# xuyuan/waymo_2d_tracking

Hardware: AMD Instinct MI355X
Metric: end-to-end frames/sec (detect+SORT) on 1920x1280 Waymo frames (higher is better)
Workload: dtype f32; 1 GPU; Cascade R-CNN X152-32x8d-FPN dconv (random-init, fp32, batch 1) on synthetic 1920x1280x3 frames -> top-100 detections/frame -> SORT (max_age 2, min_hits 0, all boxes tracked; trackers resident for the whole segment); 5 cameras x 2 frames per step per GPU; 1x1 and dense 3x3 convolutions: f32 operands as exact 3 x bf16 splits, six cross terms on the bf16 matrix cores, f32 accumulate (csrc/det_gemm_s; stage=e2e, parallelism=sequence-shard x1

## Files before the change

include/waymodet.h:

```cpp
#ifndef WAYMODET_H
#define WAYMODET_H
#include <stddef.h>
#include <stdint.h>
#ifdef __cplusplus
extern "C" {
#endif

int wd_roi_pool_fpn_f32(const float* const* feats, const int32_t* heights, const int32_t* widths,
                        const float* scales, int n_levels, int channels, int batch,
                        const float* rois, int n_rois, int pooled, int min_level, int canonical_level,
                        float canonical_size, float* out, void* stream);

size_t wd_nms_workspace(int n);
int wd_select_kept(const uint8_t* keep_mask, const uint8_t* valid, const int64_t* order, int n, int cap, int64_t* out_idx,
                   int32_t* count, void* stream);
int wd_nms_sorted_f32(const float* boxes, const int32_t* idxs, int n, float iou_threshold,
                      uint8_t* keep_mask, int32_t* n_keep, void* workspace, size_t workspace_bytes, void* stream);

size_t wd_gemm_nt_workspace(int M, int N, int K);
int wd_gemm_nt_ws_f32(const float* A, const float* Bt, const float* bias, const float* residual, int relu, int M, int N, int K,
                      float* C, void* workspace, size_t workspace_bytes, void* stream);

int wd_gemm_lt_f32(const float* a, const float* w, const float* bias, const float* residual, float* out, int m, int n, int k,
                   int relu, void* workspace, size_t workspace_bytes, void* stream);
int wd_gemm_lt_plan_info(int m, int n, int k, int relu, int has_bias, int has_residual, float* best_us, int* candidates);
size_t wd_gemm_split_packed_bytes(int N, int K);
int wd_gemm_split_pack_weight(const float* w, int N, int K, void* packed, void* stream);
int wd_gemm_split_pack_weight_strided(const float* w, int N, int K, long stride_n, long stride_k, void* packed, void* stream);
typedef struct WdSplitPackDesc {
    const float* src;
    void* dst;
    long s_n, s_c, s_kh, s_kw;
    long first_block;
    int N, K, C, ksize, flip, reserved;
} WdSplitPackDesc;
int wd_gemm_split_pack_batch(const WdSplitPackDesc* descs_device, int count, long total_blocks, void* stream);
size_t wd_gemm_split_workspace(long M, int N, int K);
int wd_gemm_split_f32(const float* a, long lda, const void* packed_w, const float* bias, const float* residual, float* out, long ldc,
                      int M, int N, int K, int relu, void* workspace, size_t workspace_bytes, void* stream);
int wd_conv_split_f32(const float* x, int batch, int H, int W, int C, const void* packed_w, int ksize, int stride, int pad, const float* bias,
                      const float* residual, float* out, int N, int relu, void* workspace, size_t workspace_bytes, void* stream);
int wd_gemm_split_supported(const float* a, long lda, const float* bias, const float* residual, const float* out, long ldc, long M, int N, int K);
int wd_conv_split_position_major(int batch, int H, int W, int ksize, int stride, int pad);
typedef struct WdSplitIO {
    const float* a;
    long lda;
    const void* a_planes;
    const float* residual;
    const void* residual_planes;
    float* out;
    void* out_planes;
    long ldc;
} WdSplitIO;
size_t wd_split_planes_bytes(long M, int K);
int wd_split_planes_pack_f32(const float* a, long lda, long M, int K, void* planes, void* stream);
int wd_split_planes_unpack_f32(const void* planes, long M, int K, float* out, long ldo, void* stream);
int wd_gemm_split_io(const WdSplitIO* io, const void* packed_w, const float* bias, int M, int N, int K, int relu, void* workspace,
                     size_t workspace_bytes, void* stream);
int wd_nms_segmented_f32(const float* boxes, const int32_t* idxs, const int32_t* seg_offsets, int n_seg, float iou_threshold,
                         uint8_t* keep_mask, int32_t* n_keep, void* workspace, size_t workspace_bytes, void* stream);

size_t wd_rpn_topk_workspace(const int* n_per_level, int n_levels, int k);
int wd_rpn_topk_decode_f32(const float* const* logits, const float* const* deltas, const float* const* anchors,
                           const int* n_per_level, int n_levels, int k, float img_h, float img_w, float scale_clamp,
                           float* out_boxes, float* out_scores, int32_t* out_group, uint8_t* out_valid, void* workspace,
                           size_t workspace_bytes, void* stream);
int wd_sort_candidates_f32(const float* boxes, const float* scores, const int32_t* group, const uint8_t* valid,
                           const uint8_t* valid2 , int n, float* out_boxes, float* out_scores, int32_t* out_group, uint8_t* out_valid, int64_t* out_order,
                           void* stream);
int wd_box_candidates_f32(const float* boxes, const float* s0, const float* s1, const float* s2, const int32_t* n_valid, int rows,
                          int num_classes, float score_thresh, float img_h, float img_w, float* out_boxes, float* out_scores,
                          int32_t* out_group, uint8_t* out_valid, int64_t* out_order, void* stream);
int wd_gather_kept_f32(const uint8_t* keep, const uint8_t* valid, const float* boxes, const float* scores, const int64_t* order,
                       int n, int cap, int num_classes, float* out_boxes, float* out_scores, int64_t* out_class, int32_t* count,
                       void* stream);
int wd_detections_to_wire(const float* boxes, const float* scores, const int64_t* classes, const int32_t* count, int n, int in_w,
                          int in_h, int hflip, int out_w, int out_h, double* xywhs, int32_t* category, void* stream);

size_t wd_deform_packed_weight_floats(int c_in, int c_out, int groups);
int wd_deform_pack_weight(const float* weight_oihw, int c_in, int c_out, int groups, float* packed, void* stream);
const char* wd_deform_conv3x3_variant(int c_in, int groups, int stride, int pad, int has_offset);
const char* wd_deform_conv3x3_last_kernel(void);
int wd_deform_conv3x3_f32(const float* x, const float* offset, const float* mask, const float* packed_weight,
                          const float* scale, const float* bias, int relu,
                          int batch, int h, int w, int c_in, int c_out, int groups, int stride, int pad,
                          float* y, void* stream);
int wd_deform_conv3x3_hint_f32(const float* x, const float* offset, const float* mask, const float* packed_weight,
                               const float* scale, const float* bias, int relu, int batch, int h, int w, int c_in,
                               int c_out, int groups, int stride, int pad, int far_offsets, float* y, void* stream);
size_t wd_deform_table_bytes(int batch, int h, int w);
int wd_deform_offsets_table_f32(const float* partial, int ld, const float* bias, int batch, int h, int w, float* offsets,
                                void* table, void* stream);
int wd_deform_conv3x3_tab_f32(const float* x, const float* offset, const float* mask, const float* packed_weight,
                              const float* scale, const float* bias, int relu, int batch, int h, int w, int c_in,
                              int c_out, int groups, int stride, int pad, int far_offsets, const void* table, float* y,
                              void* stream);

int wd_gemm_nt_f32(const float* A, const float* Bt, const float* bias, const float* residual, int relu,
                   int M, int N, int K, float* C, void* stream);

int wd_groupnorm_relu_nhwc_f32(float* x, const float* gamma, const float* beta, int n, int hw, int c, int groups,
                               float eps, int relu, void* stream);
int wd_groupnorm_relu_out_nhwc_f32(const float* x, float* y, const float* gamma, const float* beta, int n, int hw, int c, int groups,
                                   float eps, int relu, void* stream);
int wd_groupnorm_relu_bwd_nhwc_f32(const float* x, const float* dy, const float* gamma, const float* beta, int n, int hw, int c, int groups,
                                   float eps, int relu, float* dx, float* dgamma, float* dbeta, void* stream);

#define WD_LAYOUT_NCHW_F32 0
#define WD_LAYOUT_NHWC_U8 1
int wd_preprocess_out_shape(int h, int w, double scale, int divisor, int* ho, int* wo, int* hp, int* wp);
int wd_preprocess_f32(const void* src, int src_layout, int batch, int h, int w, double scale, int hflip, int vflip,
                      int swap_rb, const float* mean3, const float* std3, int divisor, float* out, void* stream);

int wd_decode_boxes_f32(const float* deltas, const float* boxes, const int64_t* index, int n, float wx, float wy, float ww,
                        float wh, float scale_clamp, float clip_w, float clip_h, float* out, void* stream);

int wd_roi_pool_fpn_bwd_f32(float* const* grad_feats, const int32_t* heights, const int32_t* widths, const float* scales,
                            int n_levels, int channels, int batch, const float* rois, int n_rois, int pooled, int min_level,
                            int canonical_level, float canonical_size, const float* grad_out, void* stream);
int wd_deform_im2col_f32(const float* x, const float* offset, int batch, int h, int w, int c, int groups, int stride, int pad,
                         float* col, void* stream);
int wd_deform_col2im_f32(const float* dcol, const float* x, const float* offset, int batch, int h, int w, int c, int groups,
                         int stride, int pad, float* dx, float* doffset, void* stream);
size_t wd_deform_bwd_tables_bytes(int batch, int h, int w, int stride);
int wd_deform_dxoff_f32(const float* x, const float* offset, const float* dy, const float* y_act, const float* scale, const float* weight, int batch,
                        int h, int w, int c, int groups, int stride, unsigned char* tables, float* packed_weight, float* dx, float* doffset,
                        void* stream);
size_t wd_deform_dw_scratch_floats(int batch, int h, int w, int c, int groups, int stride);
int wd_deform_dw_f32(const float* x, const float* offset, const float* dy, const float* y_act, const float* scale, int batch, int h, int w, int c,
                     int groups, int stride, float* scratch, float* dw, void* stream);

int wd_tap_shift_add_f32(const float* partial, int ld, int n_out, const float* bias, int batch, int h, int w, int stride,
                         float* out, void* stream);

int wd_upsample2x_nhwc_f32(const float* src, int batch, int h, int w, int c, float* dst, void* stream);

int wd_bias_relu_f32(float* y, const float* bias, long m, int n, int relu, void* stream);

int wd_act_bwd_f32(const float* dy, const float* y, const float* scale, long m, int n, int relu, float* g, void* stream);

int wd_autocontrast_u8(uint8_t* img, int h, int w, void* workspace24, void* stream);

int wd_jpeg_info(const uint8_t* data, int64_t n, int32_t* width, int32_t* height, int32_t* components, int32_t* h_samp,
                 int32_t* v_samp, int32_t* restart_interval);
int wd_jpeg_decode_rgb_u8(const uint8_t* data, int64_t n, uint8_t* rgb, int64_t capacity, int32_t* width, int32_t* height,
                          int32_t* sync_rounds, void* stream);
int wd_jpeg_last_stats(int32_t* out4);

#ifdef __cplusplus
}
#endif
#endif
```

waymo_2d_tracking_amd/csrc/det_gemm_split.hip:

```cpp
#include "common.h"
#include "../../include/waymodet.h"
#include <cstdlib>
#include <cstring>

namespace {

using bf16x8 = __attribute__((ext_vector_type(8))) __bf16;
using bf16x2 = __attribute__((ext_vector_type(2))) __bf16;
using f32x2 = __attribute__((ext_vector_type(2))) float;
using f32x16 = __attribute__((ext_vector_type(16))) float;
using u32x4 = __attribute__((ext_vector_type(4))) unsigned;

constexpr int BK = 64;
constexpr int BN = 256;
constexpr int NTHREADS = 512;
constexpr int CHUNK = 6144;

struct SplitArgs {
    const float* a;
    const unsigned char* ap;
    const uint4* w;
    const float* bias;
    const float* residual;
    const unsigned char* resp;
// ... 24 lines not shown
__device__ __forceinline__ float bf_lo(unsigned v) { return __uint_as_float(v << 16); }
__device__ __forceinline__ float bf_hi(unsigned v) { return __uint_as_float(v & 0xffff0000u); }

__device__ __forceinline__ size_t planes_offset(int row, int col, int ncols) {
    return ((size_t)(row >> 5) * (size_t)(ncols >> 5) + (size_t)(col >> 5)) * CHUNK +
           (size_t)((row & 31) * 64 + ((((col >> 3) & 3) ^ ((row >> 2) & 3)) << 4) + ((col >> 2) & 1) * 8);
}

constexpr int LDC = BN + 8;

template <int MT>
__device__ __forceinline__ void split_epilogue(const SplitArgs& p, unsigned char* smem, const f32x16 (&acc)[MT], int m0, int n0, int wave, int lane, int mlim,
                                               int row_mul = 1, int row_add = 0) {
    const int rr = lane & 31, rg = lane >> 5;
    float* ct = reinterpret_cast<float*>(smem);
    const int ncols = p.N - n0 < BN ? p.N - n0 : BN;
    constexpr int PASS = 3;
    auto stage = [&](int i0) {
        if (i0 > 0) __builtin_amdgcn_s_barrier();
#pragma unroll
        for (int i = i0; i < i0 + PASS && i < MT; ++i)
#pragma unroll
            for (int e = 0; e < 16; ++e)
                ct[((i - i0) * 32 + (e & 3) + 8 * (e >> 2) + 4 * rg) * LDC + 32 * wave + rr] = acc[i][e];
        __builtin_amdgcn_s_waitcnt(0xC07F);
        __builtin_amdgcn_s_barrier();
    };
    if (p.outp == nullptr) {
        const int c4 = 4 * lane;
        float4 bv = make_float4(0.f, 0.f, 0.f, 0.f);
        if (p.bias && c4 < ncols) bv = *reinterpret_cast<const float4*>(p.bias + n0 + c4);
        constexpr int RPW = 32 * PASS / 8;
#pragma unroll
        for (int i0 = 0; i0 < MT; i0 += PASS) {
            const int nrows = 32 * ((MT - i0) < PASS ? (MT - i0) : PASS);
            float4 rv[RPW];
            if (p.residual) {
#pragma unroll
                for (int j = 0; j < RPW; ++j) {
                    const int r = wave + 8 * j, row = m0 + 32 * i0 + r;
                    rv[j] = make_float4(0.f, 0.f, 0.f, 0.f);
                    if (r < nrows && row < mlim && c4 < ncols)
                        rv[j] = *reinterpret_cast<const float4*>(p.residual + (size_t)(row * row_mul + row_add) * p.ldc + n0 + c4);
                }
            } else if (p.resp) {
#pragma unroll
                for (int j = 0; j < RPW; ++j) {
                    const int r = wave + 8 * j, row = m0 + 32 * i0 + r;
                    rv[j] = make_float4(0.f, 0.f, 0.f, 0.f);
                    if (r < nrows && row < mlim && c4 < ncols) {
                        const unsigned char* q = p.resp + planes_offset(row * row_mul + row_add, n0 + c4, p.N);
                        const uint2 h = *reinterpret_cast<const uint2*>(q), m = *reinterpret_cast<const uint2*>(q + 2048),
                                    l = *reinterpret_cast<const uint2*>(q + 4096);
                        rv[j] = make_float4((bf_lo(h.x) + bf_lo(m.x)) + bf_lo(l.x), (bf_hi(h.x) + bf_hi(m.x)) + bf_hi(l.x),
                                            (bf_lo(h.y) + bf_lo(m.y)) + bf_lo(l.y), (bf_hi(h.y) + bf_hi(m.y)) + bf_hi(l.y));
                    }
                }
            }
            stage(i0);
#pragma unroll
            for (int j = 0; j < RPW; ++j) {
                const int r = wave + 8 * j, row = m0 + 32 * i0 + r;
                if (r < nrows && row < mlim && c4 < ncols) {
                    float4 v = *reinterpret_cast<const float4*>(ct + r * LDC + c4);
                    v.x += bv.x; v.y += bv.y; v.z += bv.z; v.w += bv.w;
                    if (p.residual || p.resp) { v.x += rv[j].x; v.y += rv[j].y; v.z += rv[j].z; v.w += rv[j].w; }
                    if (p.relu) { v.x = fmaxf(v.x, 0.f); v.y = fmaxf(v.y, 0.f); v.z = fmaxf(v.z, 0.f); v.w = fmaxf(v.w, 0.f); }
                    *reinterpret_cast<float4*>(p.out + (size_t)(row * row_mul + row_add) * p.ldc + n0 + c4) = v;
                }
            }
        }
        return;
    }
    const int ur = lane >> 2;
    constexpr int UPW = PASS * 8 * 2 / 8;
    const int ncb = ncols >> 5;
#pragma unroll
    for (int i0 = 0; i0 < MT; i0 += PASS) {
        const int nrb = (MT - i0) < PASS ? (MT - i0) : PASS;
        const int nunits = nrb * ncb * 2;
        uint4 rq[UPW][3];
#pragma unroll
        for (int j = 0; j < UPW; ++j) {
            const int u = wave + 8 * j;
            rq[j][0] = rq[j][1] = rq[j][2] = make_uint4(0u, 0u, 0u, 0u);
            if (u < nunits && m0 + 32 * (i0 + u / (2 * ncb)) < mlim) {
                const int rbi = u / (2 * ncb), cb = (u >> 1) - rbi * ncb, h = u & 1;
                const int r = 16 * h + ur, row = m0 + 32 * (i0 + rbi) + r;
                const int c8 = 8 * ((lane & 3) ^ ((r >> 2) & 3)), col = n0 + 32 * cb + c8;
                if (p.resp) {
                    const unsigned char* q = p.resp + ((size_t)(row >> 5) * (size_t)(p.N >> 5) + (size_t)(col >> 5)) * CHUNK + h * 1024 + lane * 16;
                    rq[j][0] = *reinterpret_cast<const uint4*>(q);
                    rq[j][1] = *reinterpret_cast<const uint4*>(q + 2048);
                    rq[j][2] = *reinterpret_cast<const uint4*>(q + 4096);
                } else if (p.residual && row < mlim) {
                    const uint4* q = reinterpret_cast<const uint4*>(p.residual + (size_t)row * p.ldc + col);
                    rq[j][0] = q[0];
                    rq[j][1] = q[1];
                }
            }
        }
        stage(i0);
#pragma unroll
        for (int j = 0; j < UPW; ++j) {
            const int u = wave + 8 * j;
            if (u < nunits && m0 + 32 * (i0 + u / (2 * ncb)) < mlim) {
                const int rbi = u / (2 * ncb), cb = (u >> 1) - rbi * ncb, h = u & 1;
                const int r = 16 * h + ur, row = m0 + 32 * (i0 + rbi) + r;
                const int c8 = 8 * ((lane & 3) ^ ((r >> 2) & 3)), col = n0 + 32 * cb + c8;
                const float* src = ct + (32 * rbi + r) * LDC + 32 * cb + c8;
                float4 v0 = *reinterpret_cast<const float4*>(src), v1 = *reinterpret_cast<const float4*>(src + 4);
                if (p.bias) {
                    const float4 b0 = *reinterpret_cast<const float4*>(p.bias + col), b1 = *reinterpret_cast<const float4*>(p.bias + col + 4);
                    v0.x += b0.x; v0.y += b0.y; v0.z += b0.z; v0.w += b0.w; v1.x += b1.x; v1.y += b1.y; v1.z += b1.z; v1.w += b1.w;
                }
                if (p.resp) {
                    const uint4 hh = rq[j][0], mm = rq[j][1], ll = rq[j][2];
                    v0.x += (bf_lo(hh.x) + bf_lo(mm.x)) + bf_lo(ll.x); v0.y += (bf_hi(hh.x) + bf_hi(mm.x)) + bf_hi(ll.x);
                    v0.z += (bf_lo(hh.y) + bf_lo(mm.y)) + bf_lo(ll.y); v0.w += (bf_hi(hh.y) + bf_hi(mm.y)) + bf_hi(ll.y);
                    v1.x += (bf_lo(hh.z) + bf_lo(mm.z)) + bf_lo(ll.z); v1.y += (bf_hi(hh.z) + bf_hi(mm.z)) + bf_hi(ll.z);
                    v1.z += (bf_lo(hh.w) + bf_lo(mm.w)) + bf_lo(ll.w); v1.w += (bf_hi(hh.w) + bf_hi(mm.w)) + bf_hi(ll.w);
                } else if (p.residual) {
                    const uint4 q0 = rq[j][0], q1 = rq[j][1];
                    v0.x += __uint_as_float(q0.x); v0.y += __uint_as_float(q0.y); v0.z += __uint_as_float(q0.z); v0.w += __uint_as_float(q0.w);
                    v1.x += __uint_as_float(q1.x); v1.y += __uint_as_float(q1.y); v1.z += __uint_as_float(q1.z); v1.w += __uint_as_float(q1.w);
                }
                if (p.relu) {
                    v0.x = fmaxf(v0.x, 0.f); v0.y = fmaxf(v0.y, 0.f); v0.z = fmaxf(v0.z, 0.f); v0.w = fmaxf(v0.w, 0.f);
                    v1.x = fmaxf(v1.x, 0.f); v1.y = fmaxf(v1.y, 0.f); v1.z = fmaxf(v1.z, 0.f); v1.w = fmaxf(v1.w, 0.f);
                }
                if (p.out && row < mlim) {
                    float4* d = reinterpret_cast<float4*>(p.out + (size_t)row * p.ldc + col);
                    d[0] = v0; d[1] = v1;
                }
                unsigned hv[4], mv[4], lv[4];
                split_pair(v0.x, v0.y, hv[0], mv[0], lv[0]); split_pair(v0.z, v0.w, hv[1], mv[1], lv[1]);
                split_pair(v1.x, v1.y, hv[2], mv[2], lv[2]); split_pair(v1.z, v1.w, hv[3], mv[3], lv[3]);
                unsigned char* q = p.outp + ((size_t)(row >> 5) * (size_t)(p.N >> 5) + (size_t)(col >> 5)) * CHUNK + h * 1024 + lane * 16;
                *reinterpret_cast<uint4*>(q) = make_uint4(hv[0], hv[1], hv[2], hv[3]);
                *reinterpret_cast<uint4*>(q + 2048) = make_uint4(mv[0], mv[1], mv[2], mv[3]);
                *reinterpret_cast<uint4*>(q + 4096) = make_uint4(lv[0], lv[1], lv[2], lv[3]);
            }
        }
    }
}

__device__ __forceinline__ int xcd_tile_id(int total) {
    const int x = blockIdx.x & 7, j = blockIdx.x >> 3;
    const int q = total >> 3, r = total & 7;
    if (j >= q + (x < r ? 1 : 0)) return -1;
    return (x < r ? x * (q + 1) : r * (q + 1) + (x - r) * q) + j;
}

template <int MT, int MODE>
__global__ __launch_bounds__(NTHREADS, 2) void gemm_split_kernel(const SplitArgs p) {
    extern __shared__ __attribute__((aligned(16))) unsigned char smem[];
    constexpr int BM = 32 * MT;
    constexpr int PLANE = BM * 64;
    constexpr int BUF = 3 * PLANE;
    const int tid = threadIdx.x, lane = tid & 63;
    const int wave = __builtin_amdgcn_readfirstlane(tid >> 6);
    constexpr bool CONV = MODE == 1 || MODE == 3;
    constexpr bool PM = MODE == 3;
    int id = PM ? (int)blockIdx.x : xcd_tile_id(p.tiles_m * p.tiles_n * p.splitk);
    if (id < 0 || (PM && id >= p.tiles_m * p.tiles_n)) return;
#ifdef WD_DEBUG
    long long t_start = 0, r_start = 0, t_main = 0, t_epi = 0;
    if (p.stamps) { t_start = __builtin_amdgcn_s_memtime(); r_start = __builtin_amdgcn_s_memrealtime(); }
    const int id_stamp = id;
#endif
    const int kz = PM ? 0 : id % p.splitk;
    if (!PM) id /= p.splitk;
    const int tm = id / p.tiles_n, tn = id - tm * p.tiles_n;
    int m0 = tm * BM;
    const int n0 = tn * BN;
    const int kc = CONV ? p.C / 32 : 1;
    int pm_y = 0, pm_x = 0, pm_nvt = 9;
    unsigned long long pm_taps = 0x876543210ull;
    if (PM) {
        const int nch = (p.M / (p.H * p.W) + BM - 1) / BM;
        const int wi = p.W - 2, hi = p.H - 2, ni = wi * hi, ne = 2 * wi + 2 * hi;
        int t = tm, c, q;
        if (t < ni * nch) { c = t / ni; q = t - c * ni; pm_y = 1 + q / wi; pm_x = 1 + q - (q / wi) * wi; }
        else if (t < (ni + ne) * nch) {
            t -= ni * nch; c = t / ne; q = t - c * ne;
            if (q < wi) { pm_y = 0; pm_x = 1 + q; }
            else if (q < 2 * wi) { pm_y = p.H - 1; pm_x = 1 + q - wi; }
            else if (q < 2 * wi + hi) { pm_x = 0; pm_y = 1 + q - 2 * wi; }
            else { pm_x = p.W - 1; pm_y = 1 + q - 2 * wi - hi; }
        } else { t -= (ni + ne) * nch; c = t >> 2; q = t & 3; pm_y = (q >> 1) ? p.H - 1 : 0; pm_x = (q & 1) ? p.W - 1 : 0; }
        m0 = c * BM;
        pm_taps = 0; pm_nvt = 0;
        for (int tp = 0; tp < 9; ++tp) {
            const int yy = pm_y + tp / 3 - 1, xx = pm_x + tp % 3 - 1;
            if (yy >= 0 && yy < p.H && xx >= 0 && xx < p.W) { pm_taps |= (unsigned long long)tp << (4 * pm_nvt); ++pm_nvt; }
        }
    }
    auto pm_tap = [&](int i) { return (int)((pm_taps >> (4 * i)) & 15ull); };
    const int nk_all = PM ? pm_nvt * kc : p.K / 32;
    const int per = (nk_all + p.splitk - 1) / p.splitk;
    const int k0 = kz * per;
    const int nk = (k0 + per <= nk_all) ? per : nk_all - k0;

    const int srow = tid >> 4, sk2 = tid & 15;
    unsigned aoff[MT];
    unsigned vmask[MT];
#pragma unroll
    for (int i = 0; i < MT; ++i) {
        int m = m0 + srow + 32 * i;
        if (PM) {
            const int maps = p.M / (p.H * p.W);
            m = m < maps ? m : maps - 1;
            aoff[i] = (unsigned)(((m * p.H + pm_y - 1) * p.W + pm_x - 1) * p.C + 2 * sk2);
            vmask[i] = 0x1ffu;
            continue;
        }
        m = m < p.M ? m : p.M - 1;
        if (MODE == 0) {
            aoff[i] = (unsigned)(m * p.lda) + 2u * sk2;
            vmask[i] = 1u;
        } else {
            const int hw = p.Ho * p.Wo;
            const int b = m / hw, rem = m - b * hw;
            const int yo = rem / p.Wo, xo = rem - yo * p.Wo;
            const int y0 = yo * p.stride - p.pad, x0 = xo * p.stride - p.pad;
            aoff[i] = (unsigned)(((b * p.H + y0) * p.W + x0) * p.C + 2 * sk2);
            unsigned vm = 0;
            for (int t = 0; t < p.ksize * p.ksize; ++t) {
                const int yy = y0 + t / p.ksize, xx = x0 + t % p.ksize;
                if (yy >= 0 && yy < p.H && xx >= 0 && xx < p.W) vm |= 1u << t;
            }
            vmask[i] = vm;
        }
    }
    float2 araw[MT];
    auto a_fetch = [&](int kt, int i) -> float2 {
        kt = k0 + (kt < nk ? kt : nk - 1);
        if (MODE == 0) {
            return *reinterpret_cast<const float2*>(p.a + (size_t)(aoff[i] + (unsigned)(kt * 32)));
        } else {
            const int ti = kt / kc, cb = kt - ti * kc;
            const int tap = PM ? pm_tap(ti) : ti;
            const int dy = tap / p.ksize, dx = tap - dy * p.ksize;
            const unsigned delta = (unsigned)((dy * p.W + dx) * p.C + cb * 32);
            const bool ok = ((vmask[i] >> tap) & 1u) != 0;
            const unsigned off = ok ? aoff[i] + delta : 2u * sk2;
            const float2 v = *reinterpret_cast<const float2*>(p.a + (size_t)off);
            return ok ? v : make_float2(0.f, 0.f);
        }
    };
    auto a_load_row = [&](int kt, int i) { araw[i] = a_fetch(kt, i); };
    int f_idx = 0, f_tap = 0, f_cb = 0;
    unsigned f_delta = 0;
    int f_act = 0;
    auto f_place = [&]() {
        f_act = PM ? pm_tap(f_tap) : f_tap;
        const int dy = p.ksize == 3 ? (f_act * 11) >> 5 : 0, dx = f_act - dy * p.ksize;
        f_delta = (unsigned)((dy * p.W + dx) * p.C + f_cb * 32);
    };
    auto f_set = [&](int kt) {
        f_idx = kt < nk ? kt : nk - 1;
        const int ks = k0 + f_idx;
        f_tap = ks / kc; f_cb = ks - f_tap * kc;
        f_place();
    };
    auto f_advance = [&](int kt) {
        if (kt < nk && kt > f_idx) {
            ++f_idx;
            if (++f_cb == kc) { f_cb = 0; ++f_tap; }
            f_place();
        }
    };
    auto a_fetch_cur = [&](int i) -> float2 {
        const bool ok = ((vmask[i] >> f_act) & 1u) != 0;
        const unsigned off = ok ? aoff[i] + f_delta : 2u * sk2;
        const float2 v = *reinterpret_cast<const float2*>(p.a + (size_t)off);
        return ok ? v : make_float2(0.f, 0.f);
    };
    const int wofs = srow * 64 + ((((sk2 >> 2) ^ ((srow >> 2) & 3))) << 4) + ((sk2 & 3) << 2);
    auto a_store_val = [&](int bufoff, int i, float2 v) {
        unsigned char* base = smem + bufoff + wofs + i * 2048;
        unsigned h, m, l;
        split_pair(v.x, v.y, h, m, l);
        *reinterpret_cast<unsigned*>(base) = h;
        *reinterpret_cast<unsigned*>(base + PLANE) = m;
        *reinterpret_cast<unsigned*>(base + 2 * PLANE) = l;
    };
    auto a_store_row = [&](int bufoff, int i) { a_store_val(bufoff, i, araw[i]); };

    const int nt32 = (n0 >> 5) + wave;
    const bool active = nt32 * 32 < p.N;
    const uint4* wbase = p.w + (size_t)(active ? nt32 : 0) * (size_t)(p.K / 16) * 192 + lane;
    const int nsub = nk * 2;
    bf16x8 wf[2][3];
    auto w_load = [&](int sub, int slot) {
        sub = 2 * k0 + (sub < nsub ? sub : nsub - 1);
        if (PM) {
            const int ti = sub / (2 * kc);
            sub = pm_tap(ti) * 2 * kc + (sub - ti * 2 * kc);
        }
        const uint4* q = wbase + (size_t)sub * 192;
#pragma unroll
        for (int pl = 0; pl < 3; ++pl) wf[slot][pl] = __builtin_bit_cast(bf16x8, q[pl * 64]);
    };

    f32x16 acc[MT];
#pragma unroll
    for (int i = 0; i < MT; ++i)
#pragma unroll
// ... 271 lines not shown
    d[1] = make_float4((bf_lo(h.z) + bf_lo(m.z)) + bf_lo(l.z), (bf_hi(h.z) + bf_hi(m.z)) + bf_hi(l.z), (bf_lo(h.w) + bf_lo(m.w)) + bf_lo(l.w),
                       (bf_hi(h.w) + bf_hi(m.w)) + bf_hi(l.w));
}

__global__ __launch_bounds__(256) void gemm_split_pack_kernel(const float* __restrict__ w, int N, int K, long sn, long sk, uint4* __restrict__ out, long total) {
    const long t = (long)blockIdx.x * 256 + threadIdx.x;
    if (t >= total) return;
    const int k8 = K / 8;
    const int n = (int)(t / k8), kq = (int)(t - (long)n * k8);
    float v[8];
#pragma unroll
    for (int e = 0; e < 8; ++e) v[e] = n < N ? w[(size_t)n * sn + (size_t)(8 * kq + e) * sk] : 0.f;
    unsigned h[4], m[4], l[4];
#pragma unroll
    for (int e = 0; e < 4; ++e) split_pair(v[2 * e], v[2 * e + 1], h[e], m[e], l[e]);
    const int nt = n >> 5, ks = kq >> 1, ln = (n & 31) + 32 * (kq & 1);
    uint4* dst = out + ((size_t)nt * (K / 16) + ks) * 192 + ln;
    dst[0] = make_uint4(h[0], h[1], h[2], h[3]);
    dst[64] = make_uint4(m[0], m[1], m[2], m[3]);
    dst[128] = make_uint4(l[0], l[1], l[2], l[3]);
}

__global__ __launch_bounds__(256) void gemm_split_pack_batch_kernel(const WdSplitPackDesc* __restrict__ descs, int count) {
    int lo = 0, hi = count - 1;
    const long blk = blockIdx.x;
    while (lo < hi) {
        const int mid = (lo + hi + 1) >> 1;
        if (descs[mid].first_block <= blk) lo = mid; else hi = mid - 1;
    }
    const WdSplitPackDesc d = descs[lo];
    const long t = (blk - d.first_block) * 256 + threadIdx.x;
    const int k8 = d.K / 8;
    const long total = (long)((d.N + 31) / 32) * 32 * k8;
    if (t >= total) return;
    const int n = (int)(t / k8), kq = (int)(t - (long)n * k8);
    const int k = 8 * kq, tap = k / d.C, c = k - tap * d.C;
    int kh = tap / d.ksize, kw = tap - kh * d.ksize;
    if (d.flip) { kh = d.ksize - 1 - kh; kw = d.ksize - 1 - kw; }
    const float* src = d.src + (size_t)n * d.s_n + (size_t)kh * d.s_kh + (size_t)kw * d.s_kw + (size_t)c * d.s_c;
    float v[8];
#pragma unroll
    for (int e = 0; e < 8; ++e) v[e] = n < d.N ? src[(size_t)e * d.s_c] : 0.f;
    unsigned h[4], m[4], l[4];
#pragma unroll
    for (int e = 0; e < 4; ++e) split_pair(v[2 * e], v[2 * e + 1], h[e], m[e], l[e]);
    const int nt = n >> 5, ks = kq >> 1, ln = (n & 31) + 32 * (kq & 1);
    uint4* dst = reinterpret_cast<uint4*>(d.dst) + ((size_t)nt * (d.K / 16) + ks) * 192 + ln;
    dst[0] = make_uint4(h[0], h[1], h[2], h[3]);
    dst[64] = make_uint4(m[0], m[1], m[2], m[3]);
    dst[128] = make_uint4(l[0], l[1], l[2], l[3]);
}

__global__ __launch_bounds__(256) void gemm_split_reduce_kernel(const float4* __restrict__ part, int splitk, long mn4, int n4, const float4* __restrict__ bias,
                                                                const float* __restrict__ residual, const unsigned char* __restrict__ resp, long ldc, int relu,
                                                                float* __restrict__ out, unsigned char* __restrict__ outp) {
    const long i = (long)blockIdx.x * 256 + threadIdx.x;
    if (i >= mn4) return;
    float4 v = part[i];
    for (int z = 1; z < splitk; ++z) {
        const float4 q = part[(size_t)z * mn4 + i];
        v.x += q.x; v.y += q.y; v.z += q.z; v.w += q.w;
    }
    const long row = i / n4;
    const int c4 = (int)(i - row * n4);
    if (bias) { const float4 b = bias[c4]; v.x += b.x; v.y += b.y; v.z += b.z; v.w += b.w; }
    const size_t o = (size_t)row * ldc + 4 * c4;
    if (residual) { const float4 q = *reinterpret_cast<const float4*>(residual + o); v.x += q.x; v.y += q.y; v.z += q.z; v.w += q.w; }
    if (resp) {
        const unsigned char* q = resp + planes_offset((int)row, 4 * c4, 4 * n4);
        const uint2 h = *reinterpret_cast<const uint2*>(q), m = *reinterpret_cast<const uint2*>(q + 2048), l = *reinterpret_cast<const uint2*>(q + 4096);
        v.x += (bf_lo(h.x) + bf_lo(m.x)) + bf_lo(l.x); v.y += (bf_hi(h.x) + bf_hi(m.x)) + bf_hi(l.x);
        v.z += (bf_lo(h.y) + bf_lo(m.y)) + bf_lo(l.y); v.w += (bf_hi(h.y) + bf_hi(m.y)) + bf_hi(l.y);
    }
    if (relu) { v.x = fmaxf(v.x, 0.f); v.y = fmaxf(v.y, 0.f); v.z = fmaxf(v.z, 0.f); v.w = fmaxf(v.w, 0.f); }
    if (out) *reinterpret_cast<float4*>(out + o) = v;
    if (outp) {
        unsigned h0, m0_, l0, h1, m1, l1;
        split_pair(v.x, v.y, h0, m0_, l0);
        split_pair(v.z, v.w, h1, m1, l1);
        unsigned char* q = outp + planes_offset((int)row, 4 * c4, 4 * n4);
        *reinterpret_cast<uint2*>(q) = make_uint2(h0, h1);
        *reinterpret_cast<uint2*>(q + 2048) = make_uint2(m0_, m1);
        *reinterpret_cast<uint2*>(q + 4096) = make_uint2(l0, l1);
    }
}

bool experiment_mode() {
    static const bool on = []() { const char* e = getenv("WT_EXPERIMENT"); return e && e[0] == '1'; }();
    return on;
}
int experiment_knob(const char* name) {
    const char* e = getenv(name);
    if (!e) return 0;
    if (!experiment_mode()) {
        fprintf(stderr, "libwaymotrack: %s=%s ignored (laboratory switch; set WT_EXPERIMENT=1 to use it)\n", name, e);
        return 0;
    }
    return atoi(e);
}

struct Plan { int mt, splitk; };

constexpr int MT_MIN = 4, MT_MAX = 6;

Plan pick_plan(long M, int N, int K, bool allow_split) {
    static const int forced_mt = experiment_knob("WD_SPLIT_MT");
    static const int forced_sk = experiment_knob("WD_SPLIT_SPLITK");
    const long tn = (N + BN - 1) / BN;
    const int nk_all = K / 32;
    Plan best{5, 1};
    double best_t = 1e30;
    const int mt_min = (forced_mt == 2 || forced_mt == 3) ? forced_mt : MT_MIN;
    for (int mt = MT_MAX; mt >= mt_min; --mt) {
        if (forced_mt >= 2 && forced_mt <= MT_MAX && mt != forced_mt) continue;
        const long tiles = ((M + 32 * mt - 1) / (32 * mt)) * tn;
        for (int sk = 1; sk <= 32; ++sk) {
            if (sk > 1 && !allow_split) break;
            if (forced_sk >= 1 && sk != forced_sk && allow_split) continue;
            const int per = (nk_all + sk - 1) / sk;
            if (sk > 1 && (per < 3 || (long)(sk - 1) * per >= nk_all)) continue;
            const long rounds = (tiles * sk + 255) / 256;
            const double eff = (mt == 4 || mt == 5) ? 1.0 : 1.24;
            double t = rounds * (mt * per * 0.52 * eff + 2.0 + mt);
            if (sk > 1) t += 3.0 + (double)(sk + 1) * M * N * 4.0 / 4.0e6;
            if (t < best_t * 0.97) { best_t = t; best = Plan{mt, sk}; }
        }
    }
    return best;
}

#ifdef WD_DEBUG
long long* g_stamps = nullptr;
#endif

int occupancy_guard(const void* fn, int mt) {
    hipFuncAttributes at{};
    WT_HIP(hipFuncGetAttributes(&at, fn));
    const int alloc = (at.numRegs + 7) / 8 * 8;
    int victim = 232;
    const int g = wt::victim_regs_grouped_conv(), d = wt::victim_regs_deform64();
    if (g > 0 && d > 0) victim = g < d ? g : d;
    if (2 * alloc + victim <= 512 && !experiment_mode()) {
        wt::set_error("split-operand kernel with %d row blocks was compiled to %d registers: a %d-register wave of deform_conv3x3_kernel<64> / "
                      "grouped_conv3x3_c8_kernel fits beside two of its waves on a SIMD, which is the co-residency that corrupts those kernels "
                      "(profiles/r06_costream_victim_side.txt); refused (WT_EXPERIMENT=1 overrides)", mt, at.numRegs, victim);
        return WT_ERR_INVALID;
    }
    return WT_OK;
}

template <int MT, int MODE>
int launch(const SplitArgs& a, hipStream_t stream) {
    constexpr size_t lds_epi = 32u * (MT < 3 ? MT : 3) * LDC * 4u;
    constexpr size_t lds_ring = (MODE == 2 ? 4u : 3u) * 3u * 32u * MT * 64u;
    constexpr size_t lds = lds_ring > lds_epi ? lds_ring : lds_epi;
    const void* fn = MODE == 2 ? reinterpret_cast<const void*>(gemm_split_planes_kernel<MT>)
                               : reinterpret_cast<const void*>(gemm_split_kernel<MT, MODE == 2 ? 0 : MODE>);
    static wt::OncePerDevice attr;
    const int dev = wt::device_index();
    if (attr.needed(dev)) {
        WT_TRY(occupancy_guard(fn, MT));
        WT_HIP(hipFuncSetAttribute(fn, hipFuncAttributeMaxDynamicSharedMemorySize, (int)lds));
        attr.mark(dev);
    }
    const int total = a.tiles_m * a.tiles_n * a.splitk;
    const dim3 grid((unsigned)((total + 7) / 8 * 8));
    if constexpr (MODE == 2) hipLaunchKernelGGL((gemm_split_planes_kernel<MT>), grid, dim3(NTHREADS), lds, stream, a);
    else hipLaunchKernelGGL((gemm_split_kernel<MT, MODE>), grid, dim3(NTHREADS), lds, stream, a);
    WT_HIP(hipGetLastError());
    return WT_OK;
}

template <int MODE>
int dispatch(SplitArgs& a, void* workspace, size_t workspace_bytes, hipStream_t stream) {
#ifdef WD_DEBUG
    a.stamps = g_stamps;
#endif
    const bool can_split = workspace != nullptr && (a.N % 4) == 0;
    Plan pl = pick_plan(a.M, a.N, a.K, can_split);
    if (pl.splitk > 1 && workspace_bytes < (size_t)pl.splitk * a.M * a.N * sizeof(float)) pl = pick_plan(a.M, a.N, a.K, false);
    const int mt = pl.mt;
    a.splitk = pl.splitk;
    a.part = pl.splitk > 1 ? (float*)workspace : nullptr;
    a.tiles_m = (a.M + 32 * mt - 1) / (32 * mt);
    a.tiles_n = (a.N + BN - 1) / BN;
    int rc;
    switch (mt) {
        case 2: rc = launch<2, MODE>(a, stream); break;
        case 3: rc = launch<3, MODE>(a, stream); break;
        case 4: rc = launch<4, MODE>(a, stream); break;
        case 6: rc = launch<6, MODE>(a, stream); break;
        default: rc = launch<5, MODE>(a, stream); break;
    }
    if (rc != WT_OK || a.splitk == 1) return rc;
    const long mn4 = (long)a.M * a.N / 4;
    hipLaunchKernelGGL(gemm_split_reduce_kernel, dim3((unsigned)((mn4 + 255) / 256)), dim3(256), 0, stream, (const float4*)a.part, a.splitk, mn4, a.N / 4,
                       (const float4*)a.bias, a.residual, a.resp, a.ldc, a.relu, a.out, a.outp);
    WT_HIP(hipGetLastError());
    return WT_OK;
}

int dispatch_position_major(SplitArgs& a, hipStream_t stream) {
#ifdef WD_DEBUG
    a.stamps = g_stamps;
#endif
    const int maps = a.M / (a.H * a.W), kc = a.C / 32;
    const long tn = (a.N + BN - 1) / BN;
    const long ni = (long)(a.H - 2) * (a.W - 2), ne = 2l * (a.W - 2) + 2l * (a.H - 2);
    int best = 4;
    double best_t = 1e30;
    static const int forced_mt = experiment_knob("WD_SPLIT_MT");
    for (int mt = MT_MAX; mt >= MT_MIN; --mt) {
        if (forced_mt >= MT_MIN && forced_mt <= MT_MAX && mt != forced_mt) continue;
        const long nch = (maps + 32 * mt - 1) / (32 * mt);
        const double eff = (mt == 4 || mt == 5) ? 1.0 : 1.24;
        auto tile = [&](int taps) { return mt * taps * kc * 0.52 * eff + 2.0 + mt; };
        const double work = (double)nch * tn * (ni * tile(9) + ne * tile(6) + 4 * tile(4)) / 256.0;
        const double t = work > tile(9) ? work : tile(9);
        if (t < best_t * 0.97) { best_t = t; best = mt; }
    }
    a.splitk = 1; a.part = nullptr;
    a.tiles_m = a.H * a.W * ((maps + 32 * best - 1) / (32 * best));
    a.tiles_n = (int)tn;
    switch (best) {
        case 4: return launch<4, 3>(a, stream);
        case 6: return launch<6, 3>(a, stream);
        default: return launch<5, 3>(a, stream);
    }
}

bool misaligned(const void* p) { return (reinterpret_cast<uintptr_t>(p) & 15) != 0; }

}

extern "C" {

#ifdef WD_DEBUG
int wd_gemm_split_debug_stamps(long long* buf) {
    g_stamps = buf;
    return WT_OK;
}
#endif

size_t wd_gemm_split_packed_bytes(int N, int K) {
    if (N <= 0 || K <= 0 || (K % BK)) return 0;
    return (size_t)((N + 31) / 32) * 32 * (size_t)K * 6;
}

int wd_gemm_split_pack_weight_strided(const float* w, int N, int K, long stride_n, long stride_k, void* packed, void* stream_) {
    WT_TRY(wt::ensure_device());
    if (!w || !packed || N <= 0 || K <= 0 || (K % BK)) {
        wt::set_error("wd_gemm_split_pack_weight: K must be a positive multiple of %d (N=%d K=%d)", BK, N, K);
        return WT_ERR_INVALID;
    }
    const long total = (long)((N + 31) / 32) * 32 * (K / 8);
    hipLaunchKernelGGL(gemm_split_pack_kernel, dim3((unsigned)((total + 255) / 256)), dim3(256), 0, (hipStream_t)stream_, w, N, K, stride_n, stride_k,
                       (uint4*)packed, total);
    WT_HIP(hipGetLastError());
    return WT_OK;
}

int wd_gemm_split_pack_weight(const float* w, int N, int K, void* packed, void* stream_) {
    return wd_gemm_split_pack_weight_strided(w, N, K, (long)K, 1, packed, stream_);
}

int wd_gemm_split_pack_batch(const WdSplitPackDesc* descs_device, int count, long total_blocks, void* stream_) {
    WT_TRY(wt::ensure_device());
    if (count <= 0 || total_blocks <= 0) return WT_OK;
    if (!descs_device || total_blocks >= (1l << 31)) {
        wt::set_error("wd_gemm_split_pack_batch: NULL descriptor array or too many workgroups (%ld)", total_blocks);
        return WT_ERR_INVALID;
    }
    hipLaunchKernelGGL(gemm_split_pack_batch_kernel, dim3((unsigned)total_blocks), dim3(256), 0, (hipStream_t)stream_, descs_device, count);
    WT_HIP(hipGetLastError());
    return WT_OK;
}

size_t wd_gemm_split_workspace(long M, int N, int K) {
    if (M <= 0 || N <= 0 || K <= 0 || (K % BK) || (N % 32)) return 0;
    const Plan pl = pick_plan(M, N, K, true);
    return pl.splitk > 1 ? (size_t)pl.splitk * M * N * sizeof(float) : 0;
}

int wd_gemm_split_supported(const float* a, long lda, const float* bias, const float* residual, const float* out, long ldc, long M, int N, int K) {
    return M > 0 && N > 0 && K > 0 && (K % BK) == 0 && (N % 32) == 0 && (lda & 3) == 0 && (ldc & 3) == 0 && lda >= K && ldc >= N && !misaligned(a) &&
           !misaligned(bias) && !misaligned(residual) && !misaligned(out) && M < (1l << 31) && M * lda < (1l << 31);
}

int wd_gemm_split_f32(const float* a, long lda, const void* packed_w, const float* bias, const float* residual, float* out, long ldc,
                      int M, int N, int K, int relu, void* workspace, size_t workspace_bytes, void* stream_) {
    WT_TRY(wt::ensure_device());
    if (M <= 0 || N <= 0) return WT_OK;
    if (!a || !packed_w || !out || misaligned(packed_w) || !wd_gemm_split_supported(a, lda, bias, residual, out, ldc, M, N, K)) {
        wt::set_error("wd_gemm_split_f32: needs K %% %d == 0, N %% 32 == 0, 16-byte aligned rows and M * lda < 2^31 (M=%d N=%d K=%d lda=%ld)", BK, M, N,
                      K, lda);
        return WT_ERR_INVALID;
    }
    SplitArgs s{};
    s.a = a; s.w = (const uint4*)packed_w; s.bias = bias; s.residual = residual; s.out = out;
    s.lda = lda; s.ldc = ldc; s.M = M; s.N = N; s.K = K; s.relu = relu;
    return dispatch<0>(s, workspace, workspace_bytes, (hipStream_t)stream_);
}

size_t wd_split_planes_bytes(long M, int K) {
    if (M <= 0 || K <= 0 || (K % 32)) return 0;
    return (size_t)((M + 31) / 32) * (size_t)(K / 32) * CHUNK;
}

int wd_split_planes_pack_f32(const float* a, long lda, long M, int K, void* planes, void* stream_) {
    WT_TRY(wt::ensure_device());
    if (!a || !planes || M <= 0 || M >= (1l << 31) || K <= 0 || (K % 32) || (lda & 3) || lda < K || misaligned(a) || misaligned(planes)) {
        wt::set_error("wd_split_planes_pack_f32: needs K %% 32 == 0 and 16-byte aligned rows (M=%ld K=%d lda=%ld)", M, K, lda);
        return WT_ERR_INVALID;
    }
    const long total = ((M + 31) / 32) * 32 * (K / 8);
    hipLaunchKernelGGL(split_planes_pack_kernel, dim3((unsigned)((total + 255) / 256)), dim3(256), 0, (hipStream_t)stream_, a, lda, (int)M, K,
                       (unsigned char*)planes, total);
    WT_HIP(hipGetLastError());
    return WT_OK;
}

int wd_split_planes_unpack_f32(const void* planes, long M, int K, float* out, long ldo, void* stream_) {
    WT_TRY(wt::ensure_device());
    if (!out || !planes || M <= 0 || M >= (1l << 31) || K <= 0 || (K % 32) || (ldo & 3) || ldo < K || misaligned(out) || misaligned(planes)) {
        wt::set_error("wd_split_planes_unpack_f32: needs K %% 32 == 0 and 16-byte aligned rows (M=%ld K=%d ldo=%ld)", M, K, ldo);
        return WT_ERR_INVALID;
    }
    const long total = M * (K / 8);
    hipLaunchKernelGGL(split_planes_unpack_kernel, dim3((unsigned)((total + 255) / 256)), dim3(256), 0, (hipStream_t)stream_, (const unsigned char*)planes,
                       (int)M, K, out, ldo, total);
    WT_HIP(hipGetLastError());
    return WT_OK;
}

int wd_gemm_split_io(const WdSplitIO* io, const void* packed_w, const float* bias, int M, int N, int K, int relu, void* workspace,
                     size_t workspace_bytes, void* stream_) {
    WT_TRY(wt::ensure_device());
    if (M <= 0 || N <= 0) return WT_OK;
    if (!io || !packed_w || misaligned(packed_w) || (!io->a && !io->a_planes) || (io->a && io->a_planes) || (!io->out && !io->out_planes) ||
        (io->residual && io->residual_planes) || K <= 0 || (K % BK) || (N % 32) || misaligned(io->a_planes) || misaligned(io->residual_planes) ||
        misaligned(io->out_planes) ||
        !wd_gemm_split_supported(io->a ? io->a : (const float*)packed_w, io->a ? io->lda : K, bias, io->residual, io->out, io->ldc ? io->ldc : N, M, N, K)) {
        wt::set_error("wd_gemm_split_io: exactly one of a / a_planes, at least one of out / out_planes, at most one residual form; K %% %d == 0, "
                      "N %% 32 == 0, 16-byte aligned pointers and rows (M=%d N=%d K=%d)", BK, M, N, K);
        return WT_ERR_INVALID;
    }
    SplitArgs s{};
    s.a = io->a; s.ap = (const unsigned char*)io->a_planes; s.w = (const uint4*)packed_w; s.bias = bias;
    s.residual = io->residual; s.resp = (const unsigned char*)io->residual_planes; s.out = io->out; s.outp = (unsigned char*)io->out_planes;
    s.lda = io->a ? io->lda : K; s.ldc = io->ldc ? io->ldc : N; s.M = M; s.N = N; s.K = K; s.relu = relu;
    return io->a ? dispatch<0>(s, workspace, workspace_bytes, (hipStream_t)stream_) : dispatch<2>(s, workspace, workspace_bytes, (hipStream_t)stream_);
}

int wd_conv_split_position_major(int batch, int H, int W, int ksize, int stride, int pad) {
    static const int no_pm = experiment_knob("WD_SPLIT_NO_POSMAJOR");
    return !no_pm && ksize == 3 && stride == 1 && pad == 1 && H >= 3 && W >= 3 && H * W <= 81 && batch >= 256;
}

int wd_conv_split_f32(const float* x, int batch, int H, int W, int C, const void* packed_w, int ksize, int stride, int pad, const float* bias,
                      const float* residual, float* out, int N, int relu, void* workspace, size_t workspace_bytes, void* stream_) {
    WT_TRY(wt::ensure_device());
    const int Ho = (H + 2 * pad - ksize) / stride + 1, Wo = (W + 2 * pad - ksize) / stride + 1;
    const long M = (long)batch * Ho * Wo;
    if (M <= 0 || N <= 0) return WT_OK;
    if (!x || !packed_w || !out || (ksize != 1 && ksize != 3) || stride < 1 || pad < 0 || C <= 0 || (C % BK) || (N % 32) || misaligned(x) ||
        misaligned(out) || misaligned(bias) || misaligned(residual) || (long)batch * H * W * C >= (1l << 31) || M >= (1l << 31)) {
        wt::set_error("wd_conv_split_f32: needs ksize 1 or 3, C %% %d == 0, N %% 32 == 0 and fewer than 2^31 input elements (C=%d N=%d k=%d)", BK, C, N, ksize);
        return WT_ERR_INVALID;
    }
    SplitArgs s{};
    s.a = x; s.w = (const uint4*)packed_w; s.bias = bias; s.residual = residual; s.out = out;
    s.lda = C; s.ldc = N; s.M = (int)M; s.N = N; s.K = ksize * ksize * C; s.relu = relu;
    s.H = H; s.W = W; s.C = C; s.Ho = Ho; s.Wo = Wo; s.stride = stride; s.pad = pad; s.ksize = ksize;
    if (wd_conv_split_position_major(batch, H, W, ksize, stride, pad)) return dispatch_position_major(s, (hipStream_t)stream_);
    return dispatch<1>(s, workspace, workspace_bytes, (hipStream_t)stream_);
}

}
```

Measured before the change: 42.89 frames/s.

## Add row-segment 3x3 conv kernel reusing a staged A tile across dx taps

```diff
diff --git a/include/waymodet.h b/include/waymodet.h
--- a/include/waymodet.h
+++ b/include/waymodet.h
@@ -42,6 +42,7 @@
                       const float* residual, float* out, int N, int relu, void* workspace, size_t workspace_bytes, void* stream);
 int wd_gemm_split_supported(const float* a, long lda, const float* bias, const float* residual, const float* out, long ldc, long M, int N, int K);
 int wd_conv_split_position_major(int batch, int H, int W, int ksize, int stride, int pad);
+int wd_conv_split_row_segment(int batch, int H, int W, int C, int N, int ksize, int stride, int pad, size_t workspace_bytes);
 typedef struct WdSplitIO {
     const float* a;
     long lda;
diff --git a/waymo_2d_tracking_amd/csrc/det_gemm_split.hip b/waymo_2d_tracking_amd/csrc/det_gemm_split.hip
--- a/waymo_2d_tracking_amd/csrc/det_gemm_split.hip
+++ b/waymo_2d_tracking_amd/csrc/det_gemm_split.hip
@@ -200,9 +200,173 @@
     return (x < r ? x * (q + 1) : r * (q + 1) + (x - r) * q) + j;
 }
 
+template <int MT>
+__device__ __forceinline__ void rowseg_tile(const SplitArgs& p, unsigned char* smem) {
+    constexpr int BM = 32 * MT;
+    constexpr int ZOFF = (BM + 2) * 64;
+    constexpr int PLANE = (BM + 3) * 64;
+    constexpr int BUF = 3 * PLANE;
+    constexpr int NS = MT + 1;
+    const int tid = threadIdx.x, lane = tid & 63;
+    const int wave = __builtin_amdgcn_readfirstlane(tid >> 6);
+    const int id = xcd_tile_id(p.tiles_m * p.tiles_n);
+    if (id < 0) return;
+    const int tm = id / p.tiles_n, tn = id - tm * p.tiles_n;
+    const int m0 = tm * BM, n0 = tn * BN;
+    const int Wd = p.W, Cd = p.C, npix = p.M;
+    const int kc = Cd / 32;
+    const int nk = 3 * kc;
+
+    const int srow = tid >> 4, sk2 = tid & 15;
+    const bool tail_row = srow < 2;
+    const int g0 = m0 - 1 - Wd + srow;
+    auto a_fetch = [&](int dyW, int cb32, int j) -> float2 {
+        const int g = g0 + 32 * j + dyW;
+        const int gc = g < 0 ? 0 : (g < npix ? g : npix - 1);
+        const unsigned off = (unsigned)gc * (unsigned)Cd + (unsigned)cb32 + 2u * sk2;
+        return *reinterpret_cast<const float2*>(p.a + (size_t)off);
+    };
+    const int wofs = srow * 64 + ((((sk2 >> 2) ^ ((srow >> 2) & 3))) << 4) + ((sk2 & 3) << 2);
+    auto a_store = [&](int bufoff, int j, float2 v, int dyW) {
+        if (j < MT || tail_row) {
+            unsigned char* base = smem + bufoff + wofs + j * 2048;
+            unsigned keep = (unsigned)(g0 + 32 * j + dyW) < (unsigned)npix ? 0xffffffffu : 0u;
+            asm volatile("" : "+v"(keep));
+            v.x = __uint_as_float(__float_as_uint(v.x) & keep);
+            v.y = __uint_as_float(__float_as_uint(v.y) & keep);
+            unsigned h, m, l;
+            split_pair(v.x, v.y, h, m, l);
+            *reinterpret_cast<unsigned*>(base) = h;
+            *reinterpret_cast<unsigned*>(base + PLANE) = m;
+            *reinterpret_cast<unsigned*>(base + 2 * PLANE) = l;
+        }
+    };
+    int f_idx = 0, f_dyW = 0, f_cb32 = 0;
+    int w_dyW = 0;
+    auto f_advance = [&]() {
+        w_dyW = f_dyW;
+        if (f_idx < nk - 1) {
+            ++f_idx;
+            f_cb32 += 32;
+            if (f_cb32 == Cd) { f_cb32 = 0; f_dyW += Wd; }
+        }
+    };
+
+    const int rr = lane & 31, rg = lane >> 5;
+    unsigned vmask[(MT + 2) / 3];
+#pragma unroll
+    for (int i = 0; i < (MT + 2) / 3; ++i) vmask[i] = 0u;
+#pragma unroll
+    for (int i = 0; i < MT; ++i) {
+        const int m = m0 + 32 * i + rr;
+        unsigned vm = 0;
+        if (m < npix) {
+            const int hw = p.H * Wd, rem = m - (m / hw) * hw;
+            const int y = rem / Wd, x = rem - y * Wd;
+            for (int t = 0; t < 9; ++t) {
+                const int yy = y + t / 3 - 1, xx = x + t % 3 - 1;
+                if (yy >= 0 && yy < p.H && xx >= 0 && xx < Wd) vm |= 1u << t;
+            }
+        }
+        vmask[i / 3] |= vm << (9 * (i % 3));
+    }
+    int roff[3];
+#pragma unroll
+    for (int dx = 0; dx < 3; ++dx) roff[dx] = (rr + dx) * 64 + (((rg ^ (((rr + dx) >> 2) & 3))) << 4);
+
+    const int nt32 = (n0 >> 5) + wave;
+    const bool active = nt32 * 32 < p.N;
+    const uint4* wbase = p.w + (size_t)(active ? nt32 : 0) * (size_t)(p.K / 16) * 192;
+    bf16x8 wf[2][3];
+    auto w_load = [&](int sub, int slot) {
+        const uint4* q = wbase + (size_t)sub * 192;
+#pragma unroll
+        for (int pl = 0; pl < 3; ++pl) wf[slot][pl] = __builtin_bit_cast(bf16x8, q[pl * 64 + lane]);
+    };
+
+    f32x16 acc[MT];
+#pragma unroll
+    for (int i = 0; i < MT; ++i)
+#pragma unroll
+        for (int e = 0; e < 16; ++e) acc[i][e] = 0.f;
+
+    if (tid < 144) *reinterpret_cast<unsigned*>(smem + (tid / 48) * BUF + ((tid >> 4) % 3) * PLANE + ZOFF + (tid & 15) * 4) = 0u;
+    float2 araw[NS];
+    w_load(0, 0);
+    w_load(1, 1);
+#pragma unroll
+    for (int b = 0; b < 2; ++b) {
+#pragma unroll
+        for (int j = 0; j < NS; ++j) araw[j] = a_fetch(f_dyW, f_cb32, j);
+        f_advance();
+#pragma unroll
+        for (int j = 0; j < NS; ++j) a_store(b * BUF, j, araw[j], w_dyW);
+    }
+#pragma unroll
+    for (int j = 0; j < NS; ++j) araw[j] = a_fetch(f_dyW, f_cb32, j);
+    f_advance();
+    __builtin_amdgcn_s_waitcnt(0xC07F);
+    __builtin_amdgcn_s_barrier();
+
+    bf16x8 af[MT][3];
+    int r_bit, r_off, r_zero;
+#define SB __builtin_amdgcn_sched_barrier(0)
+#define MF(pa, pb, slot)                                                                                      \
+    _Pragma("unroll") for (int i = 0; i < MT; ++i)                                                          \
+        acc[i] = __builtin_amdgcn_mfma_f32_32x32x16_bf16(af[i][pa], wf[slot][pb], acc[i], 0, 0, 0);
+#define ADDR(buf, bit, dx, s) r_bit = (bit); r_off = (buf) + (roff[(dx)] ^ ((s) << 5)); r_zero = (buf) + ZOFF;
+#define RD(pl)                                                                                                \
+    _Pragma("unroll") for (int i = 0; i < MT; ++i) {                                                        \
+        const int a_ = ((vmask[i / 3] >> (r_bit + 9 * (i % 3))) & 1u) ? r_off + i * 2048 : r_zero;            \
+        af[i][pl] = *reinterpret_cast<const bf16x8*>(smem + a_ + (pl) * PLANE);                              \
+    }
+#define STAGE(f_)                                                                                             \
+    if ((f_) % 2 == 0 && (f_) / 2 < NS) { a_store(wr, (f_) / 2, araw[(f_) / 2], w_dyW); araw[(f_) / 2] = a_fetch(f_dyW, f_cb32, (f_) / 2); }
+    ADDR(0, 0, 0, 0)
+    RD(2) RD(1) RD(0)
+    SB;
+    int cur = 0, nxt = BUF, wr = 2 * BUF;
+    int c_bit = 0, c_sub = 0;
+    int n_dy = 0, n_cb = 0;
+    for (int kt = 0; kt < nk; ++kt) {
+        int n_bit = c_bit, n_sub = c_sub;
+        if (kt + 1 < nk) {
+            if (++n_cb == kc) { n_cb = 0; ++n_dy; }
+            n_bit = 3 * n_dy;
+            n_sub = (3 * n_dy * kc + n_cb) * 2;
+        }
+#pragma unroll
+        for (int u = 0; u < 6; ++u) {
+            const int dx = u >> 1, s = u & 1;
+            if (u < 5) { ADDR(cur, c_bit + ((u + 1) >> 1), (u + 1) >> 1, (u + 1) & 1) } else { ADDR(nxt, n_bit, 0, 0) }
+            MF(2, 0, s) RD(2) SB;
+            MF(1, 1, s) STAGE(3 * u) SB;
+            MF(1, 0, s) RD(1) SB;
+            MF(0, 2, s) STAGE(3 * u + 1) SB;
+            MF(0, 1, s) STAGE(3 * u + 2) SB;
+            MF(0, 0, s) RD(0) w_load(dx < 2 ? c_sub + 2 * kc * (dx + 1) + s : n_sub + s, s); SB;
+        }
+        __builtin_amdgcn_s_waitcnt(0xC07F | (MT << 8));
+        __builtin_amdgcn_s_barrier();
+        SB;
+        const int t = cur; cur = nxt; nxt = wr; wr = t;
+        c_bit = n_bit; c_sub = n_sub;
+        f_advance();
+    }
+#undef STAGE
+#undef RD
+#undef ADDR
+#undef MF
+#undef SB
+    __builtin_amdgcn_s_waitcnt(0xC07F);
+    __builtin_amdgcn_s_barrier();
+    split_epilogue<MT>(p, smem, acc, m0, n0, wave, lane, p.M);
+}
+
 template <int MT, int MODE>
 __global__ __launch_bounds__(NTHREADS, 2) void gemm_split_kernel(const SplitArgs p) {
     extern __shared__ __attribute__((aligned(16))) unsigned char smem[];
+    if constexpr (MODE == 4) { rowseg_tile<MT>(p, smem); return; }
     constexpr int BM = 32 * MT;
     constexpr int PLANE = BM * 64;
     constexpr int BUF = 3 * PLANE;
@@ -780,7 +944,7 @@
 template <int MT, int MODE>
 int launch(const SplitArgs& a, hipStream_t stream) {
     constexpr size_t lds_epi = 32u * (MT < 3 ? MT : 3) * LDC * 4u;
-    constexpr size_t lds_ring = (MODE == 2 ? 4u : 3u) * 3u * 32u * MT * 64u;
+    constexpr size_t lds_ring = (MODE == 2 ? 4u : 3u) * 3u * (32u * MT + (MODE == 4 ? 3u : 0u)) * 64u;
     constexpr size_t lds = lds_ring > lds_epi ? lds_ring : lds_epi;
     const void* fn = MODE == 2 ? reinterpret_cast<const void*>(gemm_split_planes_kernel<MT>)
                                : reinterpret_cast<const void*>(gemm_split_kernel<MT, MODE == 2 ? 0 : MODE>);
@@ -799,20 +963,39 @@
     return WT_OK;
 }
 
+bool position_major_shape(int batch, int H, int W, int ksize, int stride, int pad) {
+    return ksize == 3 && stride == 1 && pad == 1 && H >= 3 && W >= 3 && H * W <= 81 && batch >= 256;
+}
+bool rowseg_shape(int batch, int H, int W, int C, int ksize, int stride, int pad) {
+    return ksize == 3 && stride == 1 && pad == 1 && C > 0 && (C % BK) == 0 && batch > 0 && H > 0 && W > 0 &&
+           !position_major_shape(batch, H, W, ksize, stride, pad);
+}
+
+Plan plan_for(long M, int N, int K, bool have_workspace, size_t workspace_bytes) {
+    const bool can_split = have_workspace && (N % 4) == 0;
+    Plan pl = pick_plan(M, N, K, can_split);
+    if (pl.splitk > 1 && workspace_bytes < (size_t)pl.splitk * M * N * sizeof(float)) pl = pick_plan(M, N, K, false);
+    return pl;
+}
+
+bool rowseg_plan(const Plan& pl) { return pl.splitk == 1 && (pl.mt == 4 || pl.mt == 5); }
+
 template <int MODE>
 int dispatch(SplitArgs& a, void* workspace, size_t workspace_bytes, hipStream_t stream) {
 #ifdef WD_DEBUG
     a.stamps = g_stamps;
 #endif
-    const bool can_split = workspace != nullptr && (a.N % 4) == 0;
-    Plan pl = pick_plan(a.M, a.N, a.K, can_split);
-    if (pl.splitk > 1 && workspace_bytes < (size_t)pl.splitk * a.M * a.N * sizeof(float)) pl = pick_plan(a.M, a.N, a.K, false);
+    const Plan pl = plan_for(a.M, a.N, a.K, workspace != nullptr, workspace_bytes);
     const int mt = pl.mt;
     a.splitk = pl.splitk;
     a.part = pl.splitk > 1 ? (float*)workspace : nullptr;
     a.tiles_m = (a.M + 32 * mt - 1) / (32 * mt);
     a.tiles_n = (a.N + BN - 1) / BN;
     int rc;
+    if constexpr (MODE == 1) {
+        if (rowseg_plan(pl) && rowseg_shape(a.M / (a.H * a.W), a.H, a.W, a.C, a.ksize, a.stride, a.pad))
+            return mt == 4 ? launch<4, 4>(a, stream) : launch<5, 4>(a, stream);
+    }
     switch (mt) {
         case 2: rc = launch<2, MODE>(a, stream); break;
         case 3: rc = launch<3, MODE>(a, stream); break;
@@ -982,7 +1165,12 @@
 
 int wd_conv_split_position_major(int batch, int H, int W, int ksize, int stride, int pad) {
     static const int no_pm = experiment_knob("WD_SPLIT_NO_POSMAJOR");
-    return !no_pm && ksize == 3 && stride == 1 && pad == 1 && H >= 3 && W >= 3 && H * W <= 81 && batch >= 256;
+    return !no_pm && position_major_shape(batch, H, W, ksize, stride, pad);
+}
+
+int wd_conv_split_row_segment(int batch, int H, int W, int C, int N, int ksize, int stride, int pad, size_t workspace_bytes) {
+    if (N <= 0 || !rowseg_shape(batch, H, W, C, ksize, stride, pad)) return 0;
+    return rowseg_plan(plan_for((long)batch * H * W, N, 9 * C, workspace_bytes > 0, workspace_bytes));
 }
 
 int wd_conv_split_f32(const float* x, int batch, int H, int W, int C, const void* packed_w, int ksize, int stride, int pad, const float* bias,
```

Result: no change. 43.25 frames/s (median of 6 runs) (+0.8%).
